# hannes-holey/GaPFlow

Measured on AMD Instinct MI355X. Metric: Mcell-updates/s (fp64), 4096^2 grid, higher is better.
Workload: dtype f64; 1 GPU; 2D journal bearing 4096x4096, fixed DH EOS, all-periodic, adaptive CFL 0.5 (BASELINE.json configs[2]); slabs=1

## Files before the change

gapflow_amd/csrc/api.hip:

```cpp
#include <hip/hip_runtime.h>
#include <algorithm>
#include <cmath>
#include <cstdio>
#include <cstdlib>
#include <cstring>
#include <map>
#include <mutex>
#include <string>
#include <tuple>
#include <vector>

#include "../../include/gapflow_hip.h"
#include "phys_setup.hpp"
#include "step_kernel.hip"
#include "aux_kernels.hip"
#include "step2_kernel.hip"
#include "gp_kernels.hip"
#include "elastic_kernels.hip"
#include "probe_kernels.hip"
#include "small_kernel.hip"
#include "profile_kernels.hip"
#include "checkpoint_kernels.hip"

using namespace gpf;
// ... 90 lines not shown
             double2* greens = nullptr; double2* spec = nullptr; double* dense = nullptr;
             double* u_prev = nullptr; double* h0 = nullptr; double* deformation = nullptr; } el;
    struct { bool on = false; int px = 0, py = 0, nky = 0, nranks = 1, relative = 0;
             int row0 = 0, nrows = 0, k0 = 0, nk = 0, nret = 0, nrows_all = 0, nmain = 0, main_g0 = 0, seam_side = -1, seam_g0 = 0, ref_row = -1;
             double alpha = 1.0, scale = 1.0;
             void* plan_y = nullptr; void* plan_x = nullptr; void* plan_yb = nullptr; int nxg = 0, g_lo = 0;
             double* dense = nullptr; double2* spec = nullptr; double2* send1 = nullptr; double2* recv1 = nullptr; double2* xspec = nullptr;
             double2* greens = nullptr; double2* send2 = nullptr; double2* recv2 = nullptr; double2* line = nullptr; double* ureal = nullptr;
             double* u_prev = nullptr; double* h0 = nullptr; double* deformation = nullptr; double* ref = nullptr; int* rows_all = nullptr; } els;
    double* gptile = nullptr;
    size_t gptile_doubles = 0;
    void* blas = nullptr;
    bool step_open = false;
    int open_parity = 0;
    bool has_q = false, has_topo = false, pre_run_done = false;
    bool prev_state_valid = false;
    long long fields_step = -1;
    bool fields_restored = false;
    long long host_step = 0;
    long long next_step = 0;
    Strip2Geom geom2[2];
    int nchunks2 = 0, nblocks2 = 0, npartials2_cap = 0, nblock_partials_cap = 0;
    bool plan2_valid = false;
    int nt_policy2 = 0;
    int keep_rows2 = 0;
    StepState* st_trial = nullptr;
    double* plan_master = nullptr;
    char plan2_note[400] = "";
};

static int enter(gpf_handle* h, bool reads_only) {
    HIP_TRY(hipSetDevice(h->cfg.device));
    if (!reads_only) { h->gp_state_mean_valid = false; h->fields_restored = false; }
    return GPF_OK;
}

static void make_phys(const gpf_config& c, Phys& P) {
    setup_phys(P, c.U, c.V, c.eta, c.zeta, c.dx, c.dy, c.eos, c.eos_par, c.piezo, c.piezo_par, c.thinning, c.thinning_par);
}

static int blocks_for(long long n, int bs = 256, int cap = 4096) {
    long long b = (n + bs - 1) / bs;
    return (int)std::max<long long>(1, std::min<long long>(b, cap));
}

#ifdef GPF_ONLY_EOS_DH
#define EOS_DISPATCH(eos, ...)                                                                          \
    do {                                                                                                \
        if ((eos) == GPF_EOS_DH) { constexpr int EOS_ = EOS_DH; __VA_ARGS__; }       \
    } while (0)
#else
// ... 62 lines not shown
    if (cfg->eos != GPF_EOS_DH) return fail(GPF_ERR_INVALID, "gpf_create: this build (-DGPF_ONLY_EOS_DH) holds the Dowson-Higginson kernels only");
#endif
    int ndev = 0;
    if (hipGetDeviceCount(&ndev) != hipSuccess || ndev == 0)
        return fail(GPF_ERR_NO_DEVICE, "gpf_create: no HIP device visible (this library has no CPU path)");
    if (cfg->device < 0 || cfg->device >= ndev) return fail(GPF_ERR_INVALID, "gpf_create: device ordinal out of range");
    HIP_TRY(hipSetDevice(cfg->device));

    gpf_handle* h = new gpf_handle();
    h->cfg = *cfg;
    Layout& L = h->L;
    L.Nx = cfg->Nx; L.Ny = cfg->Ny; L.off = 15;
    L.pitch = ((cfg->Ny + 2 + L.off + 15) / 16) * 16;
    if (const char* s = std::getenv("GPF_PITCH_PAD")) L.pitch += (std::atoi(s) / 16) * 16;
    L.plane = (long long)(cfg->Nx + 2) * L.pitch;
    if (const char* s = std::getenv("GPF_PLANE_PAD")) L.plane += (std::atoll(s) & ~1ll);
    for (int e = 0; e < 4; ++e) {
        for (int c = 0; c < 3; ++c) h->E.rule[e][c] = cfg->bc_rule[e][c];
        h->E.value[e] = cfg->bc_value[e];
    }
    h->E.halo[0] = cfg->halo_lo; h->E.halo[1] = cfg->halo_hi;
    h->split_edges = std::getenv("GPF_STEP_UNFUSED_EDGES") != nullptr;
    if (const char* s = std::getenv("GPF_ROWCOEF_TABLE")) h->rowcoef_table = std::atoi(s) != 0;
    h->gp_reuse_state_mean = std::getenv("GPF_GP_NO_STATE_MEAN") == nullptr;
    make_phys(*cfg, h->P);

    const size_t plane_b = (size_t)L.plane * sizeof(double);
    auto cleanup = [&](int code) { gpf_destroy(h); return code; };
#define HIP_TRY_C(expr)                                                                                 \
    do {                                                                                                \
        hipError_t e_ = (expr);                                                                         \
        if (e_ != hipSuccess)                                                                           \
            return cleanup(fail(GPF_ERR_HIP, std::string(#expr) + ": " + hipGetErrorString(e_)));      \
    } while (0)
    h->field_bytes = (3 * plane_b + PLANE_PAD_BYTES + 255) & ~(size_t)255;
    for (int b = 0; b < 2; ++b) {
        HIP_TRY_C(field_malloc((void**)&h->q[b], h->field_bytes));
        if (field_zero(0, h->q[b], h->field_bytes) != GPF_OK) { gpf_destroy(h); return GPF_ERR_HIP; }
    }
    HIP_TRY_C(field_malloc((void**)&h->topo, h->field_bytes));
    if (field_zero(0, h->topo, h->field_bytes) != GPF_OK) { gpf_destroy(h); return GPF_ERR_HIP; }
    HIP_TRY_C(hipDeviceSynchronize());
    const size_t g1n = (size_t)3 * L.pitch + (size_t)3 * (L.Nx + 2);
    HIP_TRY_C(hipMalloc(&h->g1, g1n * sizeof(double)));
    HIP_TRY_C(hipMemset(h->g1, 0, g1n * sizeof(double)));
    HIP_TRY_C(hipMalloc(&h->st, sizeof(StepState)));
// ... 413 lines not shown
    RowCoef* fresh = nullptr;
    if (source == 1) {
        HIP_TRY(hipMalloc(&fresh, (size_t)(n + 4) * sizeof(RowCoef)));
        HIP_TRY(hipMemsetAsync(fresh, 0, (size_t)(n + 4) * sizeof(RowCoef), h->stream));
        const double* col = h->topo + L.off + 1;
        hipLaunchKernelGGL(k_row_coef_table, dim3((n + 255) / 256), dim3(256), 0, h->stream, col, col + L.plane, (long long)L.pitch, n, h->P, fresh);
        for (int e = 0; e < 2; ++e) {
            if (!h->has_seam[e]) continue;
            const double* t = h->seam + (size_t)e * 8 * L.pitch + L.off + 1;
            hipLaunchKernelGGL(k_row_coef_table, dim3(1), dim3(64), 0, h->stream, t, t + L.pitch, 4ll * L.pitch, 2, h->P, fresh + n + 2 * e);
        }
        src = fresh;
    }
    hipError_t e = hipGetLastError();
    if (e == hipSuccess) e = hipMemcpyAsync(host, src, count * sizeof(double), hipMemcpyDeviceToHost, h->stream);
    if (e == hipSuccess) e = hipStreamSynchronize(h->stream);
    if (fresh) hipFree(fresh);
    if (e != hipSuccess) return fail(GPF_ERR_HIP, std::string("gpf_row_coefficients: ") + hipGetErrorString(e));
    return GPF_OK;
}

typedef void (*step2_kernel_t)(const Step2Args, const Phys);

static step2_kernel_t step2_kernel(int eos, bool has_ls, bool piezo, int D, int topo_mode) {
    step2_kernel_t k = nullptr;
    EOS_DISPATCH(eos, {
        if (piezo) {
            if (has_ls) k = D > 0 ? k_step2<EOS_, true, true, 1, 0> : k_step2<EOS_, true, true, -1, 0>;
            else k = D > 0 ? k_step2<EOS_, false, true, 1, 0> : k_step2<EOS_, false, true, -1, 0>;
        } else if (has_ls) {
            k = D > 0 ? k_step2<EOS_, true, false, 1, 0> : k_step2<EOS_, true, false, -1, 0>;
        } else if (topo_mode == 1) {
            k = D > 0 ? k_step2<EOS_, false, false, 1, 1> : k_step2<EOS_, false, false, -1, 1>;
        } else if (topo_mode == 2) {
            k = D > 0 ? k_step2<EOS_, false, false, 1, 2> : k_step2<EOS_, false, false, -1, 2>;
        } else if (topo_mode == 3) {
            k = D > 0 ? k_step2<EOS_, false, false, 1, 3> : k_step2<EOS_, false, false, -1, 3>;
        } else if (topo_mode == 4) {
            k = D > 0 ? k_step2<EOS_, false, false, 1, 4> : k_step2<EOS_, false, false, -1, 4>;
        } else {
            k = D > 0 ? k_step2<EOS_, false, false, 1, 0> : k_step2<EOS_, false, false, -1, 0>;
        }
    });
    return k;
}

static Strip2Geom strip2_geom(const Layout& L, int D) {
    Strip2Geom G;
// ... 77 lines not shown
    Step2Args a2;
    fill_step2_args(h, a2, D, honor_stop, log_base, slab_out, p2p);
    const bool slab = slab_out != nullptr;
    FinishArgs f;
    f.partials = h->partials; f.st = h->st;
    f.log = h->log; f.log_base = log_base; f.log_cap = h->log_cap; f.out = slab_out; f.honor_stop = honor_stop;
    f.L = L; f.E = h->E;
    f.p2p = p2p_args(h, p2p);
    f.arrive = h->arrive; f.msg = slab ? h->halo : nullptr;
    f.nstep_partials = np_step; f.block_partials = h->block_partials;
    GhostFillArgs gf;
    gf.qa = h->q[0]; gf.qb = h->q[1]; gf.st = h->st;
    gf.L = L; gf.E = h->E; gf.honor_stop = honor_stop;

    const int ntiles = (L.Nx + L.Ny + 63) / 64;
    const dim3 ggrid(std::min(ntiles, 512));
    const int nsend = slab ? std::min((6 * L.pitch + 1023) / 1024, 256) : 0;
    WaitArgs w;
    w.qa = h->q[0]; w.qb = h->q[1]; w.st = h->st; w.log = h->log; w.log_base = log_base; w.log_cap = h->log_cap;
    w.L = L; w.E = h->E; w.honor_stop = honor_stop; w.arrive = h->arrive + 1; w.timeout_ticks = h->p2p_timeout_ticks; w.p2p = f.p2p;
    w.gathered = nullptr; w.msg_len = 0; w.nranks = 0; w.rank_lo = w.rank_hi = -1; w.stage1 = fused ? 0 : 1;
    const bool has_ls = h->Ls != nullptr;
    if (fused) {
        const step2_kernel_t k2 = step2_kernel(h->cfg.eos, h->Ls != nullptr, h->cfg.piezo != 0, D, topo_mode_of(h));
        if (ev0) hipEventRecord(ev0, h->stream);
        hipLaunchKernelGGL(k2, dim3(h->nblocks2), dim3(256), 0, h->stream, a2, h->P);
        if (ev1) hipEventRecord(ev1, h->stream);
        if (p2p) {
            const dim3 cgrid(SLAB_COMMIT_BLOCKS);
            EOS_DISPATCH(h->cfg.eos, {
                hipLaunchKernelGGL((k_begin_slab<EOS_, false, false, false, true>), cgrid, dim3(256), 0, h->stream, g, w, h->P);
            });
        }
        h->g1_ready = false;
        HIP_TRY(hipGetLastError());
        return GPF_OK;
    }
    EOS_DISPATCH(h->cfg.eos, {
        if (!h->g1_ready) {
            if (topo_xonly(h)) hipLaunchKernelGGL((k_ghost_stage1<EOS_, false, false, true>), ggrid, dim3(256), 0, h->stream, g, h->P);
            else LS_PIEZO_DISPATCH(has_ls, h->cfg.piezo != 0, hipLaunchKernelGGL((k_ghost_stage1<EOS_, LS_, PZ_, false>), ggrid, dim3(256), 0, h->stream, g, h->P));
        }
        if (ev0) hipEventRecord(ev0, h->stream);
        hipLaunchKernelGGL(step2_kernel(h->cfg.eos, h->Ls != nullptr, h->cfg.piezo != 0, D, topo_mode_of(h)), dim3(h->nblocks2), dim3(256), 0, h->stream, a2, h->P);
        if (ev1) hipEventRecord(ev1, h->stream);
        hipLaunchKernelGGL((k_ghost_fill<EOS_>), dim3(h->nghost_blocks + nsend), dim3(256), 0, h->stream, gf, f, h->nghost_blocks, h->P);
        if (p2p) {
            if (topo_xonly(h)) hipLaunchKernelGGL((k_begin_slab<EOS_, false, false, true, true>), ggrid, dim3(256), 0, h->stream, g, w, h->P);
            else LS_PIEZO_DISPATCH(has_ls, h->cfg.piezo != 0, hipLaunchKernelGGL((k_begin_slab<EOS_, LS_, PZ_, false, true>), ggrid, dim3(256), 0, h->stream, g, w, h->P));
        }
    });
    h->g1_ready = p2p;
    HIP_TRY(hipGetLastError());
    return GPF_OK;
}

#include "api_probes.inc"

static bool small_grid_eligible(gpf_handle* h) {
    static const bool off = getenv("GPF_SMALL_GRID") && atoi(getenv("GPF_SMALL_GRID")) == 0;
    const long long nc = (long long)(h->L.Nx + 2) * (h->L.Ny + 2);
    return !off && nc * SMALL_DOUBLES_PER_CELL * 8 <= 150 * 1024 && h->cfg.thinning == GPF_THINNING_NONE && !h->E.halo[0] && !h->E.halo[1] &&
           !h->gp[0].set && !h->gp[1].set && !h->gp[2].set && !h->el.on;
}

static int enqueue_small_steps(gpf_handle* h, int nsteps, int honor_stop, long long log_base) {
    const Layout& L = h->L;
// ... 101 lines not shown
```

gapflow_amd/csrc/api_plan.inc:

```

constexpr int K2_LONG_MARCH_ROWS = 100;

static int plan_apply(gpf_handle* h, int nchunks, int nt, int keep = 0) {
    const Layout& L = h->L;
    const int nstrips = std::max(h->geom2[0].nstrips, h->geom2[1].nstrips);
    nchunks = std::max(1, std::min(nchunks, std::max(1, L.Nx / 4)));
    h->nchunks2 = nchunks;
    h->nt_policy2 = nt;
    h->keep_rows2 = nt >= 1 ? std::max(0, std::min(7, keep)) : 0;
    const int nwaves = nstrips * nchunks;
    h->nblocks2 = (((nwaves + 3) / 4) + 7) / 8 * 8;
    if (nwaves > h->npartials2_cap) {
        if (h->partials) HIP_TRY(hipFree(h->partials));
        h->partials = nullptr;
        HIP_TRY(hipMalloc(&h->partials, (size_t)nwaves * sizeof(Partial)));
        HIP_TRY(hipMemset(h->partials, 0, (size_t)nwaves * sizeof(Partial)));
        h->npartials2_cap = nwaves;
    }
    if (h->nblocks2 > h->nblock_partials_cap) {
        const int cap = std::max(1024, h->nblocks2);
        if (h->block_partials) HIP_TRY(hipFree(h->block_partials));
        h->block_partials = nullptr;
        HIP_TRY(hipMalloc(&h->block_partials, (size_t)cap * sizeof(Partial)));
        h->nblock_partials_cap = cap;
    }
    return GPF_OK;
}

static void fill_step2_args(gpf_handle* h, Step2Args& a2, int D, int honor_stop, long long log_base, double* slab_out, bool p2p);

static int plan_trial(gpf_handle* h, int D, float* us, int reps = 6, bool both = false) {
    static const int parity_value[2] = {0, 1};
    if (!h->st_trial) HIP_TRY(hipMalloc(&h->st_trial, sizeof(StepState)));
    h->prev_state_valid = false;
    both = both && h->plan_master != nullptr;
    int par = 0;
    if (both) GPF_TRY(current_parity(h, &par));
    Step2Args a2;
    fill_step2_args(h, a2, D, 0, 0, nullptr, false);
    a2.st = h->st_trial; a2.log = nullptr;
    const step2_kernel_t k2 = step2_kernel(h->cfg.eos, h->Ls != nullptr, h->cfg.piezo != 0, D, topo_mode_of(h));
    hipEvent_t e0, e1;
    HIP_TRY(hipEventCreate(&e0)); HIP_TRY(hipEventCreate(&e1));
    float total = 0.f;
    for (int r = -1; r < reps; ++r) {
        HIP_TRY(hipMemcpyAsync(h->st_trial, h->st, sizeof(StepState), hipMemcpyDeviceToDevice, h->stream));
        if (both && ((r + 1) & 1))
            HIP_TRY(hipMemcpyAsync(&h->st_trial->parity, &parity_value[par ^ 1], sizeof(int), hipMemcpyHostToDevice, h->stream));
        HIP_TRY(hipEventRecord(e0, h->stream));
        hipLaunchKernelGGL(k2, dim3(h->nblocks2), dim3(256), 0, h->stream, a2, h->P);
        HIP_TRY(hipEventRecord(e1, h->stream));
        HIP_TRY(hipEventSynchronize(e1));
        float ms = 0.f;
        HIP_TRY(hipEventElapsedTime(&ms, e0, e1));
        if (r >= 0) total += ms;
    }
    hipEventDestroy(e0); hipEventDestroy(e1);
    if (both) GPF_TRY(field_copy(h->stream, h->q[par], h->plan_master, h->field_bytes));
    HIP_TRY(hipGetLastError());
    *us = total / reps * 1e3f;
    return GPF_OK;
}

static float placement_best_seen(const gpf_handle* h, int D, float mine) {
// ... 109 lines not shown
        }
        h->topo = best_home;
    }
    GPF_TRY(trial(bi, bj, &us, true));
    HIP_TRY(hipStreamSynchronize(h->stream));
    for (double* b : rest) field_free(b);
    h->q[par] = pool[bi]; h->q[par ^ 1] = pool[bj];
    return GPF_OK;
}

static const char* const NT_NAME[3] = {"plain loads and stores", "non-temporal stores", "non-temporal loads and stores"};
constexpr int K2_KEEP_ROWS_DEFAULT = 4;
static const int K2_KEEP_CANDIDATES[2] = {3, 4};
static std::string keep_note(const gpf_handle* h) {
    if (h->nt_policy2 < 1) return "";
    char buf[64];
    std::snprintf(buf, sizeof buf, ", keep %d/8 rows on-die", h->keep_rows2);
    return buf;
}
static const char* coef_note(const gpf_handle* h) {
    const int topo = topo_mode_of(h);
    return topo == 4 ? ", row coefficients from the table" : topo == 3 ? ", row coefficients evaluated in the kernel" : "";
}
static int plan_step2(gpf_handle* h, int D) {
    if (h->plan2_valid) return GPF_OK;
    const Layout& L = h->L;
    h->geom2[0] = strip2_geom(L, 1);
    h->geom2[1] = strip2_geom(L, -1);
    const int nstrips = std::max(h->geom2[0].nstrips, h->geom2[1].nstrips);
    int per_cu = 0, ncu = 0;
    HIP_TRY(hipOccupancyMaxActiveBlocksPerMultiprocessor(&per_cu, (const void*)step2_kernel(h->cfg.eos, h->Ls != nullptr, h->cfg.piezo != 0, 1, topo_mode_of(h)), 256, 0));
    HIP_TRY(hipDeviceGetAttribute(&ncu, hipDeviceAttributeMultiprocessorCount, h->cfg.device));
    const int all_resident = std::max(1, std::max(1, per_cu * ncu) * 4 / nstrips);
    const int one_per_simd = (ncu * 4) / nstrips;
    const double streamed = (double)L.plane * 8.0 * (6 + (topo_mode_of(h) == 0 ? 3 : 0) + (h->Ls ? 1 : 0));
    const bool nt_possible = streamed > 192.0 * 1024 * 1024;
    const char* env_chunks = std::getenv("GPF_CHUNKS");
    const char* env_nt = std::getenv("GPF_NT") ? std::getenv("GPF_NT") : std::getenv("GPF_NT_STORES");
    const char* env_tune = std::getenv("GPF_PLAN_TUNE");
    int nchunks = all_resident;
    if (one_per_simd >= 1 && L.Nx / one_per_simd >= K2_LONG_MARCH_ROWS) nchunks = one_per_simd;
    int nt = nt_possible ? 2 : 0;
    if (env_chunks && std::atoi(env_chunks) > 0) nchunks = std::atoi(env_chunks);
    if (env_nt) nt = std::max(0, std::min(2, std::atoi(env_nt)));
    const char* env_keep = std::getenv("GPF_KEEP_ROWS");
    int keep = nt_possible ? K2_KEEP_ROWS_DEFAULT : 0;
    if (env_keep) keep = std::max(0, std::min(7, std::atoi(env_keep)));
    const bool tune = !(env_tune && std::atoi(env_tune) == 0) && !h->split_edges && h->pre_run_done && (long long)L.Nx * L.Ny >= (1ll << 20) &&
                      one_per_simd >= 1 && L.Nx / one_per_simd >= 16 && !(env_chunks && env_nt);
    if (!tune) {
        GPF_TRY(plan_apply(h, nchunks, nt, keep));
        std::snprintf(h->plan2_note, sizeof h->plan2_note, "%d chunks per strip, %s%s%s (rule of thumb%s)", h->nchunks2,
                      NT_NAME[h->nt_policy2], coef_note(h), keep_note(h).c_str(), (env_chunks || env_nt || env_keep) ? ", pinned by the environment" : "");
        h->plan2_valid = true;
        return GPF_OK;
    }
    std::string placement_note;
    GPF_TRY(plan_apply(h, nchunks, nt));
    {
        int par = 0;
        GPF_TRY(current_parity(h, &par));
        if (field_malloc((void**)&h->plan_master, h->field_bytes) == hipSuccess)
            GPF_TRY(field_copy(h->stream, h->plan_master, h->q[par], h->field_bytes));
        else { (void)hipGetLastError(); h->plan_master = nullptr; }
    }
    {
        float unused = 0.f;
        const double step_s = 1.1e-11 * (double)L.Nx * L.Ny + 1e-5;
        GPF_TRY(plan_trial(h, D, &unused, (int)std::min(200.0, std::max(8.0, 0.012 / step_s))));
    }
    float best = 0.f;
    int best_chunks = nchunks;
    int best_nt = nt;
    int best_keep = 0;
    std::string seen, keep_seen;
    auto pick_plan = [&]() -> int {
        best = 0.f;
        seen.clear();
        for (int c : {one_per_simd, all_resident}) {
            if (env_chunks && std::atoi(env_chunks) > 0) c = std::atoi(env_chunks);
            for (int pol = 0; pol < (nt_possible && !env_nt ? 3 : 1); ++pol) {
                const int cand_nt = env_nt ? nt : pol;
                GPF_TRY(plan_apply(h, c, cand_nt));
                float us = 0.f;
                GPF_TRY(plan_trial(h, D, &us, 6, true));
                char buf[48];
                std::snprintf(buf, sizeof buf, " %d/%s %.0f", h->nchunks2, cand_nt == 2 ? "nt" : cand_nt == 1 ? "nts" : "plain", us);
                seen += buf;
                if (best == 0.f || us < best) { best = us; best_chunks = c; best_nt = cand_nt; }
            }
            if ((env_chunks && std::atoi(env_chunks) > 0) || one_per_simd == all_resident) break;
        }
        best_keep = 0;
        keep_seen.clear();
        if (best_nt >= 1) {
            if (env_keep) best_keep = keep;
            else if (nt_possible) {
                char buf[48];
                std::snprintf(buf, sizeof buf, " 0 %.0f", best);
                keep_seen = buf;
                float best_k = best;
                for (int k : K2_KEEP_CANDIDATES) {
                    GPF_TRY(plan_apply(h, best_chunks, best_nt, k));
                    float us = 0.f;
                    GPF_TRY(plan_trial(h, D, &us, 6, true));
                    std::snprintf(buf, sizeof buf, ", %d %.0f", k, us);
                    keep_seen += buf;
                    if (us < best_k) { best_k = us; best_keep = k; }
                }
            }
        }
        return plan_apply(h, best_chunks, best_nt, best_keep);
    };
    const bool verify = std::getenv("GPF_PLACEMENT_PRINT") && std::atoi(std::getenv("GPF_PLACEMENT_PRINT")) >= 2;
    auto stamp = [&](const char* when) {
        if (!verify) return;
        int par = 0;
        if (current_parity(h, &par) != GPF_OK) return;
        std::fprintf(stderr, "[gpf] %-28s q[par] %p %016llx   master %p %016llx\n", when, (void*)h->q[par], field_checksum(h->stream, h->q[par], h->field_bytes),
                     (void*)h->plan_master, h->plan_master ? field_checksum(h->stream, h->plan_master, h->field_bytes) : 0ull);
    };
    stamp("before the first plan");
    GPF_TRY(pick_plan());
    stamp("after the first plan");
    const std::string first_seen = seen;
    GPF_TRY(plan_placement(h, D, placement_note));
    stamp("after the placement");
    if (!placement_note.empty()) GPF_TRY(pick_plan());
    stamp("after the second plan");
    HIP_TRY(hipStreamSynchronize(h->stream));
    field_free(h->plan_master);
    h->plan_master = nullptr;
    GPF_TRY(plan_apply(h, best_chunks, best_nt, best_keep));
    const std::string kept = keep_note(h) + (keep_seen.empty() ? (env_keep && h->nt_policy2 >= 1 ? " (pinned by the environment)" : "")
                                                               : " (timed, us: k" + keep_seen + ")");
    std::snprintf(h->plan2_note, sizeof h->plan2_note, "%d chunks per strip, %s%s%s (timed, us:%s;%s%s%s)", h->nchunks2,
                  NT_NAME[h->nt_policy2], coef_note(h), kept.c_str(), seen.c_str(), placement_note.c_str(),
                  placement_note.empty() ? "" : "; before the placement:", placement_note.empty() ? "" : first_seen.c_str());
    DBG("plan_step2: %s", h->plan2_note);
    h->plan2_valid = true;
    return GPF_OK;
}

extern "C" const char* gpf_plan_note(gpf_handle* h) { return h ? h->plan2_note : ""; }
```

gapflow_amd/csrc/step2_kernel.hip:

```cpp
#include <hip/hip_runtime.h>
#include "device_types.hpp"

namespace gpf {

constexpr int STRIP2 = 126;
#ifndef GPF_K2_AHEAD
#define GPF_K2_AHEAD 2
#endif
#ifndef GPF_K2_AHEAD_LINE
#define GPF_K2_AHEAD_LINE 4
#endif
#ifndef GPF_K2_MINWAVES
#define GPF_K2_MINWAVES 2
#endif
#ifndef GPF_K2_MINWAVES_LINE
#define GPF_K2_MINWAVES_LINE GPF_K2_MINWAVES
#endif
template <int EOS, bool HAS_LS, bool PIEZO>
struct Step2Weight {
    static constexpr bool heavy = EOS == EOS_PL || EOS == EOS_MT || EOS == EOS_BWR || EOS == EOS_BAYADA || (HAS_LS && PIEZO);
};

struct Strip2Geom {
    int w0;
// ... 61 lines not shown
template <int N>
__device__ __forceinline__ void asm_wait3(dpair& a, dpair& b, dpair& c) {
    asm volatile("s_waitcnt vmcnt(%3)" : "+v"(a), "+v"(b), "+v"(c) : "n"(N) : "memory");
}
template <int N>
__device__ __forceinline__ void asm_wait1(dpair& a) {
    asm volatile("s_waitcnt vmcnt(%1)" : "+v"(a) : "n"(N) : "memory");
}

__device__ __forceinline__ double uniform_load(const double* p) {
    typedef const __attribute__((address_space(4))) double* cptr;
    return *(cptr)(unsigned long long)p;
}

__device__ __forceinline__ RowCoef uniform_load_coef(const RowCoef* p) {
    typedef double d8 __attribute__((ext_vector_type(8)));
    typedef const __attribute__((address_space(4))) d8* cptr;
    const d8 v = *(cptr)(unsigned long long)p;
    RowCoef r;
    r.A = v[0]; r.B = v[1]; r.C = v[2]; r.S0 = v[3]; r.S1a = v[4]; r.S1b = v[5]; r.S2a = v[6]; r.S2b = v[7];
    return r;
}

template <int TOPO, bool HAS_LS>
struct RawRow {
    dpair q[3];
    dpair t[TOPO == 0 ? 3 : 1];
    dpair ls[HAS_LS ? 1 : 1];
    double th, thx, thy;
};

struct Row2 { double rho[2], jx[2], jy[2], h[2], hx[2], hy[2], Ls[2]; };

template <int EOS>
struct Red {
    double ekin, v2, c2;
    int flags;
    __device__ __forceinline__ void init() { ekin = 0.0; v2 = 0.0; c2 = (EOS == EOS_DH) ? __builtin_inf() : 0.0; flags = 0; }
    __device__ __forceinline__ void cell(double r, double jx, double jy, double w, const Phys& P) {
        const double v = (jx * jx + jy * jy) * rcp(r);
        ekin += w * (v * 0.5);
        v2 = fmax(v2, v);
        if (v != v) flags |= 1;
        if (r < 0.0) flags |= 2;
        if (EOS == EOS_DH) {
            c2 = fmin(c2, fabs(P.e[7] - r));
        } else {
            const double c = eos_c2<EOS>(r, P);
            if (!(c >= 0.0)) flags |= 4;
            c2 = fmax(c2, c);
        }
    }
};

template <int EOS, bool HAS_LS, bool PIEZO, int D, int TOPO>
__device__ __forceinline__ void step_strip2(const Step2Args& a, const Phys& P, const double* __restrict__ qin,
                                            double* __restrict__ qout, int strip, int chunk, int lane,
                                            double (*stash)[128], Acc& result) {
    const Layout L = a.L;
    const Strip2Geom G = a.G;
    const bool fused = (a.fused & 1) != 0;
    const int policy = __builtin_amdgcn_readfirstlane(a.fused);

    const bool y_periodic = a.E.rule[2][0] == BC_P;
    const bool ghost_strip = strip == G.s_ghost;
    const bool wrap_strip = fused && y_periodic && ghost_strip;
    const bool wrap_lane = wrap_strip && (lane == G.lane_wrap || lane == G.lane_wrap + 1);
    const int ma = wrap_lane ? G.wrap_ma + 2 * (lane - G.lane_wrap) : G.w0 + strip * STRIP2 + 2 * lane;
    const int iy_lo_raw = D > 0 ? ma : L.Ny - ma;
    const bool lane_ok = iy_lo_raw >= -1 && iy_lo_raw <= L.Ny + 1;
    const int iy_lo = lane_ok ? iy_lo_raw : -1;
    const int iy0 = D > 0 ? iy_lo : iy_lo + 1, iy1 = D > 0 ? iy_lo + 1 : iy_lo;
    const bool out0 = lane_ok && !wrap_lane && lane >= 1 && ma >= 1 && ma <= L.Ny;
    const bool out1 = lane_ok && !wrap_lane && lane <= 62 && ma + 1 >= 1 && ma + 1 <= L.Ny;
    const bool is_ghost_lane = ghost_strip && lane == G.lane_ghost;
    const int gsrc_lane = y_periodic ? G.wrap_src_lane : (G.slot_ghost ? G.lane_ghost : G.lane_ghost - 1);
    const int gsrc_slot = y_periodic ? G.wrap_src_slot : (G.slot_ghost ? 0 : 1);

// ... 78 lines not shown
                         : "v"(a0), "v"(a1), "v"(a2), "v"(a3), "v"(a4), "v"(a5), [nt] "s"(policy & 4) : "memory", "scc");
        } else if constexpr (HAS_LS) {
            const double* const a3 = (dummy ? lane_q : lane_ls) + rb;
            asm volatile(GPF_ROW_HEAD GPF_LD(0, 4) GPF_LD(1, 5) GPF_LD(2, 6) GPF_LD(3, 7) GPF_ROW_MID
                         GPF_LDNT(0, 4) GPF_LDNT(1, 5) GPF_LDNT(2, 6) GPF_LDNT(3, 7) GPF_ROW_TAIL
                         : "=&v"(r.q[0]), "=&v"(r.q[1]), "=&v"(r.q[2]), "=&v"(r.ls[0])
                         : "v"(a0), "v"(a1), "v"(a2), "v"(a3), [nt] "s"(policy & 4) : "memory", "scc");
        } else {
            asm volatile(GPF_ROW_HEAD GPF_LD(0, 3) GPF_LD(1, 4) GPF_LD(2, 5) GPF_ROW_MID GPF_LDNT(0, 3) GPF_LDNT(1, 4) GPF_LDNT(2, 5) GPF_ROW_TAIL
                         : "=&v"(r.q[0]), "=&v"(r.q[1]), "=&v"(r.q[2])
                         : "v"(a0), "v"(a1), "v"(a2), [nt] "s"(policy & 4) : "memory", "scc");
        }
#undef GPF_LD
#undef GPF_LDNT
#undef GPF_ROW_HEAD
#undef GPF_ROW_MID
#undef GPF_ROW_TAIL
        if (TOPO == 1 || TOPO == 3) {
            r.th = uniform_load(a.topo_line + ix); r.thx = uniform_load(a.topo_line + (L.Nx + 2) + ix);
            r.thy = TOPO == 1 ? uniform_load(a.topo_line + 2 * (L.Nx + 2) + ix) : 0.0;
        }
    };
    constexpr bool HEAVY = Step2Weight<EOS, HAS_LS, PIEZO>::heavy;
    constexpr int AHEAD_ROWS = PIEZO ? 1 : ((TOPO == 3 || TABLE) ? (HEAVY ? 2 : GPF_K2_AHEAD_LINE) : GPF_K2_AHEAD);
#ifndef GPF_K2_COUNT_STORES
#define GPF_K2_COUNT_STORES 1
#endif
    const bool stores_every_row = GPF_K2_COUNT_STORES && __builtin_amdgcn_ballot_w64(out0 || out1) != 0ull;
    auto arrive = [&](Raw& r, const int n) {
        constexpr int LOOSE = AHEAD_ROWS * NL, EXACT = AHEAD_ROWS * (NL + 3);
        static_assert(EXACT <= 63, "vmcnt is a 6-bit counter");
        const int exact = __builtin_amdgcn_readfirstlane((stores_every_row && n > n_first + AHEAD_ROWS) ? 1 : 0);
#define GPF_WAIT_ROW "s_cmp_lg_u32 %[ex], 0\n\ts_cbranch_scc1 .Lgpf_exact_%=\n\ts_waitcnt vmcnt(%[loose])\n.Lgpf_exact_%=:\n\ts_waitcnt vmcnt(%[exact])"
        if constexpr (TOPO == 0 && HAS_LS)
            asm volatile(GPF_WAIT_ROW : "+v"(r.q[0]), "+v"(r.q[1]), "+v"(r.q[2]), "+v"(r.t[0]), "+v"(r.t[1]), "+v"(r.t[2]), "+v"(r.ls[0])
                         : [ex] "s"(exact), [loose] "n"(LOOSE), [exact] "n"(EXACT) : "memory", "scc");
        else if constexpr (TOPO == 0)
            asm volatile(GPF_WAIT_ROW : "+v"(r.q[0]), "+v"(r.q[1]), "+v"(r.q[2]), "+v"(r.t[0]), "+v"(r.t[1]), "+v"(r.t[2])
                         : [ex] "s"(exact), [loose] "n"(LOOSE), [exact] "n"(EXACT) : "memory", "scc");
        else if constexpr (HAS_LS)
            asm volatile(GPF_WAIT_ROW : "+v"(r.q[0]), "+v"(r.q[1]), "+v"(r.q[2]), "+v"(r.ls[0])
                         : [ex] "s"(exact), [loose] "n"(LOOSE), [exact] "n"(EXACT) : "memory", "scc");
        else
            asm volatile(GPF_WAIT_ROW : "+v"(r.q[0]), "+v"(r.q[1]), "+v"(r.q[2])
                         : [ex] "s"(exact), [loose] "n"(LOOSE), [exact] "n"(EXACT) : "memory", "scc");
#undef GPF_WAIT_ROW
    };
// ... 200 lines not shown
                }
                const int ixo = D > 0 ? n - 1 : L.Nx + 2 - n;
                const long long rbo = (long long)ixo * L.pitch;
#if GPF_K2_NT & 2
                const bool store_nt = (policy & 2) && (ixo & 7) >= ((policy >> 3) & 7);
#endif
                auto st16 = [&](double* __restrict__ rowp, double va, double vb) {
                    dpair v;
                    v.x = D > 0 ? va : vb; v.y = D > 0 ? vb : va;
                    dpair* p = reinterpret_cast<dpair*>(reinterpret_cast<char*>(rowp) + lane_bytes);
#if GPF_K2_NT & 2
                    asm volatile("s_cmp_lg_u32 %[nt], 0\n\ts_cbranch_scc1 .Lgpf_stnt_%=\n\t"
                                 "global_store_dwordx4 %0, %1, off\n\ts_branch .Lgpf_stdone_%=\n"
                                 ".Lgpf_stnt_%=:\n\tglobal_store_dwordx4 %0, %1, off nt\n"
                                 ".Lgpf_stdone_%=:\n\ts_nop 0"
                                 :: "v"(p), "v"(v), [nt] "s"(__builtin_amdgcn_readfirstlane(store_nt ? 1 : 0)) : "memory", "scc");
#else
                    *p = v;
#endif
                };
                auto st8 = [&](double* __restrict__ rowp, unsigned int bytes, double v) {
                    *reinterpret_cast<double*>(reinterpret_cast<char*>(rowp) + bytes) = v;
                };
                if (out0 && out1) {
                    st16(qo0 + rbo, o[0][0], o[1][0]); st16(qo1 + rbo, o[0][1], o[1][1]); st16(qo2 + rbo, o[0][2], o[1][2]);
                } else if (out0) {
                    const unsigned int b = (unsigned int)(L.off + iy0) * 8u;
                    st8(qo0 + rbo, b, o[0][0]); st8(qo1 + rbo, b, o[0][1]); st8(qo2 + rbo, b, o[0][2]);
                } else if (out1) {
                    const unsigned int b = (unsigned int)(L.off + iy1) * 8u;
                    st8(qo0 + rbo, b, o[1][0]); st8(qo1 + rbo, b, o[1][1]); st8(qo2 + rbo, b, o[1][2]);
                }
                const double w = 1.0 + (ixo == seam_row_lo ? 1.0 : 0.0) + (ixo == seam_row_hi ? 1.0 : 0.0);
                if (out0) red.cell(o[0][0], o[0][1], o[0][2], w, P);
                if (out1) red.cell(o[1][0], o[1][1], o[1][2], w, P);
            }
            for (int k = 0; k < 2; ++k) {
                part[k][0] = (cur.rho[k] + q1[k][0]) - dt * (-cx * q1[k][1] + cy * (dn[k][0] - gy[k][0]) - g[k].s0);
                part[k][1] = (cur.jx[k] + q1[k][1]) - dt * (-cx * g[k].fx1 + cy * (dn[k][1] - gy[k][1]) - g[k].s1);
                part[k][2] = (cur.jy[k] + q1[k][2]) - dt * (-cx * g[k].fx2 + cy * (dn[k][2] - gy[k][2]) - g[k].s2);
            }
        }
        if (TABLE) rc_row = coef_of(n + 1);
    };
    for (int n = n_first - 1;;) {
        march(n, rowbuf[0], rowbuf[AHEAD]); if (++n > n_last + 1) break;
        march(n, rowbuf[1], rowbuf[0]); if (++n > n_last + 1) break;
// ... 84 lines not shown
            }
        }
        if (a.p2p.on) asm volatile("s_waitcnt vmcnt(0)" ::: "memory");
    }
#endif

    for (int s = 32; s >= 1; s >>= 1) {
        red.ekin += __shfl_down(red.ekin, s);
        red.v2 = fmax(red.v2, __shfl_down(red.v2, s));
        const double oc = __shfl_down(red.c2, s);
        red.c2 = (EOS == EOS_DH) ? fmin(red.c2, oc) : fmax(red.c2, oc);
        red.flags |= __shfl_down(red.flags, s);
    }
    if (EOS == EOS_DH) {
        const double it = rcp(red.c2);
        red.c2 = (red.c2 == __builtin_inf()) ? 0.0 : P.e[6] * (it * it);
    }
#ifdef GPF_K2_NO_POSTPASS
    red.flags = 0;
#endif
    result.ekin = red.ekin; result.v2 = red.v2; result.c2 = red.c2; result.mass = 0.0; result.flags = red.flags;
}

template <int EOS, bool HAS_LS, bool PIEZO, int D, int TOPO>
__global__ __launch_bounds__(256, (Step2Weight<EOS, HAS_LS, PIEZO>::heavy ? 1 : ((TOPO == 1 || TOPO == 3 || TOPO == 4) ? GPF_K2_MINWAVES_LINE : GPF_K2_MINWAVES)))
void k_step2(const Step2Args a, const Phys P) {
    __shared__ double stash[4][3][128];
    __shared__ Acc red_sm[4];
    __shared__ int s_last;
    if (halted(a.st, a.honor_stop)) return;
    if (predictor_direction(a.st) != D) __builtin_trap();
    const int par = a.st->parity;
    const double* qin = par ? a.qb : a.qa;
    double* qout = const_cast<double*>(par ? a.qa : a.qb);

    const int nb = gridDim.x;
    const int lb = (int)(blockIdx.x & 7) * (nb >> 3) + (int)(blockIdx.x >> 3);
    const int wv = __builtin_amdgcn_readfirstlane(threadIdx.x >> 6), lane = threadIdx.x & 63;
    const int w = lb * 4 + wv;
    const int strip = w % a.G.nstrips, chunk = w / a.G.nstrips;
    const bool active = chunk < a.nchunks;

    Acc own;
    own.zero();
    if (active) step_strip2<EOS, HAS_LS, PIEZO, D, TOPO>(a, P, qin, qout, strip, chunk, lane, stash[wv], own);

    if (!(a.fused & 1)) {
        if (active && lane == 0) {
            Partial p;
            p.ekin = own.ekin; p.vmax2 = own.v2; p.c2max = own.c2; p.flags = (double)own.flags;
            a.partials[w] = p;
        }
        return;
    }
#ifdef GPF_K2_NO_FINISH
    if (blockIdx.x == 0 && threadIdx.x == 0) commit_step(a.st, own.ekin + 1.0, own.v2, own.c2, own.flags, a.log, a.log_base, a.log_cap);
    return;
#endif
    if (lane == 0) red_sm[wv] = own;
    __syncthreads();
    if (threadIdx.x == 0) {
        Acc tot = red_sm[0];
        for (int i = 1; i < 4; ++i) { tot.ekin += red_sm[i].ekin; tot.v2 = fmax(tot.v2, red_sm[i].v2); tot.c2 = fmax(tot.c2, red_sm[i].c2); tot.flags |= red_sm[i].flags; }
        publish_partial(a.block_partials + blockIdx.x, tot);
        const unsigned int t = __hip_atomic_fetch_add(a.arrive, 1u, GPF_ORDER_ARRIVE, __HIP_MEMORY_SCOPE_AGENT);
        s_last = (t == (unsigned int)nb - 1) ? 1 : 0;
        if (s_last) __hip_atomic_store(a.arrive, 0u, __ATOMIC_RELAXED, __HIP_MEMORY_SCOPE_AGENT);
    }
// ... 7 lines not shown
```

Measured before the change: 122,800 Mcell-updates/s.

## Add three-waves-per-SIMD step2 kernel variant and include it in autotuning

Adds a variant of the step2 kernel with a launch-bounds minimum of three waves per SIMD, for the light x-only-gap topology modes. It shortens the row lookahead and rebuilds the output pointers from one wave-uniform base to save registers. The planner adds this form to the timed candidates, with a chunk count chosen to avoid power-of-two aliasing. It also loosens the tuning threshold. Higher occupancy is meant to hide memory latency better, at the risk of register spills or less lookahead.

```diff
diff --git a/gapflow_amd/csrc/api.hip b/gapflow_amd/csrc/api.hip
--- a/gapflow_amd/csrc/api.hip
+++ b/gapflow_amd/csrc/api.hip
@@ -136,11 +136,13 @@
     Strip2Geom geom2[2];
     int nchunks2 = 0, nblocks2 = 0, npartials2_cap = 0, nblock_partials_cap = 0;
     bool plan2_valid = false;
+    int waves2 = 0;
+    int waves_pin = 0;
     int nt_policy2 = 0;
     int keep_rows2 = 0;
     StepState* st_trial = nullptr;
     double* plan_master = nullptr;
-    char plan2_note[400] = "";
+    char plan2_note[640] = "";
 };
 
 static int enter(gpf_handle* h, bool reads_only) {
@@ -249,6 +251,7 @@
     h->E.halo[0] = cfg->halo_lo; h->E.halo[1] = cfg->halo_hi;
     h->split_edges = std::getenv("GPF_STEP_UNFUSED_EDGES") != nullptr;
     if (const char* s = std::getenv("GPF_ROWCOEF_TABLE")) h->rowcoef_table = std::atoi(s) != 0;
+    if (const char* s = std::getenv("GPF_K2_WAVES")) h->waves_pin = std::max(0, std::min(3, std::atoi(s)));
     h->gp_reuse_state_mean = std::getenv("GPF_GP_NO_STATE_MEAN") == nullptr;
     make_phys(*cfg, h->P);
 
@@ -708,8 +711,21 @@
 
 typedef void (*step2_kernel_t)(const Step2Args, const Phys);
 
-static step2_kernel_t step2_kernel(int eos, bool has_ls, bool piezo, int D, int topo_mode) {
+template <int EOS, int D, int TOPO>
+static step2_kernel_t step2_kernel_three_waves() {
+    if constexpr (Step2Weight<EOS, false, false>::heavy) return nullptr;
+    else return k_step2<EOS, false, false, D, TOPO, 3>;
+}
+
+static step2_kernel_t step2_kernel(int eos, bool has_ls, bool piezo, int D, int topo_mode, int waves = 0) {
     step2_kernel_t k = nullptr;
+    if (waves == 3 && !has_ls && !piezo && (topo_mode == 3 || topo_mode == 4)) {
+        EOS_DISPATCH(eos, {
+            if (topo_mode == 3) k = D > 0 ? step2_kernel_three_waves<EOS_, 1, 3>() : step2_kernel_three_waves<EOS_, -1, 3>();
+            else k = D > 0 ? step2_kernel_three_waves<EOS_, 1, 4>() : step2_kernel_three_waves<EOS_, -1, 4>();
+        });
+        if (k) return k;
+    }
     EOS_DISPATCH(eos, {
         if (piezo) {
             if (has_ls) k = D > 0 ? k_step2<EOS_, true, true, 1, 0> : k_step2<EOS_, true, true, -1, 0>;
@@ -833,7 +849,7 @@
     w.gathered = nullptr; w.msg_len = 0; w.nranks = 0; w.rank_lo = w.rank_hi = -1; w.stage1 = fused ? 0 : 1;
     const bool has_ls = h->Ls != nullptr;
     if (fused) {
-        const step2_kernel_t k2 = step2_kernel(h->cfg.eos, h->Ls != nullptr, h->cfg.piezo != 0, D, topo_mode_of(h));
+        const step2_kernel_t k2 = step2_kernel(h->cfg.eos, h->Ls != nullptr, h->cfg.piezo != 0, D, topo_mode_of(h), h->waves2);
         if (ev0) hipEventRecord(ev0, h->stream);
         hipLaunchKernelGGL(k2, dim3(h->nblocks2), dim3(256), 0, h->stream, a2, h->P);
         if (ev1) hipEventRecord(ev1, h->stream);
@@ -853,7 +869,7 @@
             else LS_PIEZO_DISPATCH(has_ls, h->cfg.piezo != 0, hipLaunchKernelGGL((k_ghost_stage1<EOS_, LS_, PZ_, false>), ggrid, dim3(256), 0, h->stream, g, h->P));
         }
         if (ev0) hipEventRecord(ev0, h->stream);
-        hipLaunchKernelGGL(step2_kernel(h->cfg.eos, h->Ls != nullptr, h->cfg.piezo != 0, D, topo_mode_of(h)), dim3(h->nblocks2), dim3(256), 0, h->stream, a2, h->P);
+        hipLaunchKernelGGL(step2_kernel(h->cfg.eos, h->Ls != nullptr, h->cfg.piezo != 0, D, topo_mode_of(h), h->waves2), dim3(h->nblocks2), dim3(256), 0, h->stream, a2, h->P);
         if (ev1) hipEventRecord(ev1, h->stream);
         hipLaunchKernelGGL((k_ghost_fill<EOS_>), dim3(h->nghost_blocks + nsend), dim3(256), 0, h->stream, gf, f, h->nghost_blocks, h->P);
         if (p2p) {
diff --git a/gapflow_amd/csrc/api_plan.inc b/gapflow_amd/csrc/api_plan.inc
--- a/gapflow_amd/csrc/api_plan.inc
+++ b/gapflow_amd/csrc/api_plan.inc
@@ -4,7 +4,9 @@
 static int plan_apply(gpf_handle* h, int nchunks, int nt, int keep = 0) {
     const Layout& L = h->L;
     const int nstrips = std::max(h->geom2[0].nstrips, h->geom2[1].nstrips);
-    nchunks = std::max(1, std::min(nchunks, std::max(1, L.Nx / 4)));
+    const char* const env_pinned = std::getenv("GPF_CHUNKS");
+    const int min_rows = (env_pinned && std::atoi(env_pinned) > 0) ? 3 : 4;
+    nchunks = std::max(1, std::min(nchunks, std::max(1, L.Nx / min_rows)));
     h->nchunks2 = nchunks;
     h->nt_policy2 = nt;
     h->keep_rows2 = nt >= 1 ? std::max(0, std::min(7, keep)) : 0;
@@ -39,7 +41,7 @@
     Step2Args a2;
     fill_step2_args(h, a2, D, 0, 0, nullptr, false);
     a2.st = h->st_trial; a2.log = nullptr;
-    const step2_kernel_t k2 = step2_kernel(h->cfg.eos, h->Ls != nullptr, h->cfg.piezo != 0, D, topo_mode_of(h));
+    const step2_kernel_t k2 = step2_kernel(h->cfg.eos, h->Ls != nullptr, h->cfg.piezo != 0, D, topo_mode_of(h), h->waves2);
     hipEvent_t e0, e1;
     HIP_TRY(hipEventCreate(&e0)); HIP_TRY(hipEventCreate(&e1));
     float total = 0.f;
@@ -195,6 +197,15 @@
     const int topo = topo_mode_of(h);
     return topo == 4 ? ", row coefficients from the table" : topo == 3 ? ", row coefficients evaluated in the kernel" : "";
 }
+static bool chunks_alias(const Layout& L, int nchunks) {
+    if (nchunks < 2 || L.Nx % nchunks != 0) return false;
+    const double mib = (double)(L.Nx / nchunks) * L.pitch * 8.0 / (1024.0 * 1024.0);
+    if (mib < 0.98) return false;
+    const double p2 = std::exp2(std::round(std::log2(mib)));
+    return std::fabs(mib - p2) <= 0.02 * p2;
+}
+static const char* form_note(const gpf_handle* h) { return h->waves2 == 3 ? ", three-wave form" : ", one- / two-wave form"; }
+
 static int plan_step2(gpf_handle* h, int D) {
     if (h->plan2_valid) return GPF_OK;
     const Layout& L = h->L;
@@ -206,6 +217,18 @@
     HIP_TRY(hipDeviceGetAttribute(&ncu, hipDeviceAttributeMultiprocessorCount, h->cfg.device));
     const int all_resident = std::max(1, std::max(1, per_cu * ncu) * 4 / nstrips);
     const int one_per_simd = (ncu * 4) / nstrips;
+    const int topo = topo_mode_of(h);
+    const step2_kernel_t k3 = step2_kernel(h->cfg.eos, h->Ls != nullptr, h->cfg.piezo != 0, 1, topo, 3);
+    const bool has_three = k3 != step2_kernel(h->cfg.eos, h->Ls != nullptr, h->cfg.piezo != 0, 1, topo);
+    int three_resident = 0;
+    if (has_three) {
+        int per_cu3 = 0;
+        HIP_TRY(hipOccupancyMaxActiveBlocksPerMultiprocessor(&per_cu3, (const void*)k3, 256, 0));
+        three_resident = std::max(1, std::max(1, per_cu3 * ncu) * 4 / nstrips);
+        while (three_resident > 1 && chunks_alias(L, three_resident)) --three_resident;
+    }
+    const int pin = (h->waves_pin == 3 && !has_three) ? 0 : h->waves_pin;
+    const char* const pin_ignored = (h->waves_pin == 3 && !has_three) ? ", GPF_K2_WAVES=3 ignored: this kernel has no three-wave form" : "";
     const double streamed = (double)L.plane * 8.0 * (6 + (topo_mode_of(h) == 0 ? 3 : 0) + (h->Ls ? 1 : 0));
     const bool nt_possible = streamed > 192.0 * 1024 * 1024;
     const char* env_chunks = std::getenv("GPF_CHUNKS");
@@ -214,17 +237,22 @@
     int nchunks = all_resident;
     if (one_per_simd >= 1 && L.Nx / one_per_simd >= K2_LONG_MARCH_ROWS) nchunks = one_per_simd;
     int nt = nt_possible ? 2 : 0;
+    h->waves2 = pin == 3 ? 3 : 0;
+    if (pin == 1 && one_per_simd >= 1) nchunks = one_per_simd;
+    else if (pin == 2) nchunks = all_resident;
+    else if (pin == 3) nchunks = three_resident;
     if (env_chunks && std::atoi(env_chunks) > 0) nchunks = std::atoi(env_chunks);
     if (env_nt) nt = std::max(0, std::min(2, std::atoi(env_nt)));
     const char* env_keep = std::getenv("GPF_KEEP_ROWS");
     int keep = nt_possible ? K2_KEEP_ROWS_DEFAULT : 0;
     if (env_keep) keep = std::max(0, std::min(7, std::atoi(env_keep)));
     const bool tune = !(env_tune && std::atoi(env_tune) == 0) && !h->split_edges && h->pre_run_done && (long long)L.Nx * L.Ny >= (1ll << 20) &&
-                      one_per_simd >= 1 && L.Nx / one_per_simd >= 16 && !(env_chunks && env_nt);
+                      one_per_simd >= 1 && L.Nx / one_per_simd >= 8 && !(env_chunks && env_nt);
     if (!tune) {
         GPF_TRY(plan_apply(h, nchunks, nt, keep));
-        std::snprintf(h->plan2_note, sizeof h->plan2_note, "%d chunks per strip, %s%s%s (rule of thumb%s)", h->nchunks2,
-                      NT_NAME[h->nt_policy2], coef_note(h), keep_note(h).c_str(), (env_chunks || env_nt || env_keep) ? ", pinned by the environment" : "");
+        std::snprintf(h->plan2_note, sizeof h->plan2_note, "%d chunks per strip%s, %s%s%s (rule of thumb%s%s)", h->nchunks2, form_note(h),
+                      NT_NAME[h->nt_policy2], coef_note(h), keep_note(h).c_str(), (env_chunks || env_nt || env_keep || pin) ? ", pinned by the environment" : "",
+                      pin_ignored);
         h->plan2_valid = true;
         return GPF_OK;
     }
@@ -246,24 +274,37 @@
     int best_chunks = nchunks;
     int best_nt = nt;
     int best_keep = 0;
+    int best_waves = h->waves2;
     std::string seen, keep_seen;
+    std::vector<std::pair<int, int>> forms;
+    {
+        const int fixed = env_chunks ? std::atoi(env_chunks) : 0;
+        auto add = [&](int c, int waves) {
+            const std::pair<int, int> f(fixed > 0 ? fixed : c, waves);
+            if (std::find(forms.begin(), forms.end(), f) == forms.end()) forms.push_back(f);
+        };
+        if (pin == 0 || pin == 1) add(one_per_simd, 0);
+        if (pin == 0 || pin == 2) add(all_resident, 0);
+        if (has_three && (pin == 0 || pin == 3)) add(three_resident, 3);
+    }
     auto pick_plan = [&]() -> int {
         best = 0.f;
         seen.clear();
-        for (int c : {one_per_simd, all_resident}) {
-            if (env_chunks && std::atoi(env_chunks) > 0) c = std::atoi(env_chunks);
+        for (const std::pair<int, int>& form : forms) {
+            const int c = form.first;
+            h->waves2 = form.second;
             for (int pol = 0; pol < (nt_possible && !env_nt ? 3 : 1); ++pol) {
                 const int cand_nt = env_nt ? nt : pol;
                 GPF_TRY(plan_apply(h, c, cand_nt));
                 float us = 0.f;
                 GPF_TRY(plan_trial(h, D, &us, 6, true));
                 char buf[48];
-                std::snprintf(buf, sizeof buf, " %d/%s %.0f", h->nchunks2, cand_nt == 2 ? "nt" : cand_nt == 1 ? "nts" : "plain", us);
+                std::snprintf(buf, sizeof buf, " %d%s/%s %.0f", h->nchunks2, form.second == 3 ? "w3" : "", cand_nt == 2 ? "nt" : cand_nt == 1 ? "nts" : "plain", us);
                 seen += buf;
-                if (best == 0.f || us < best) { best = us; best_chunks = c; best_nt = cand_nt; }
+                if (best == 0.f || us < best) { best = us; best_chunks = c; best_nt = cand_nt; best_waves = form.second; }
             }
-            if ((env_chunks && std::atoi(env_chunks) > 0) || one_per_simd == all_resident) break;
-        }
+        }
+        h->waves2 = best_waves;
         best_keep = 0;
         keep_seen.clear();
         if (best_nt >= 1) {
@@ -304,12 +345,14 @@
     HIP_TRY(hipStreamSynchronize(h->stream));
     field_free(h->plan_master);
     h->plan_master = nullptr;
+    h->waves2 = best_waves;
     GPF_TRY(plan_apply(h, best_chunks, best_nt, best_keep));
     const std::string kept = keep_note(h) + (keep_seen.empty() ? (env_keep && h->nt_policy2 >= 1 ? " (pinned by the environment)" : "")
                                                                : " (timed, us: k" + keep_seen + ")");
-    std::snprintf(h->plan2_note, sizeof h->plan2_note, "%d chunks per strip, %s%s%s (timed, us:%s;%s%s%s)", h->nchunks2,
+    std::snprintf(h->plan2_note, sizeof h->plan2_note, "%d chunks per strip%s, %s%s%s (timed, us:%s;%s%s%s)%s%s", h->nchunks2, form_note(h),
                   NT_NAME[h->nt_policy2], coef_note(h), kept.c_str(), seen.c_str(), placement_note.c_str(),
-                  placement_note.empty() ? "" : "; before the placement:", placement_note.empty() ? "" : first_seen.c_str());
+                  placement_note.empty() ? "" : "; before the placement:", placement_note.empty() ? "" : first_seen.c_str(),
+                  pin ? " (waves per SIMD pinned by the environment)" : "", pin_ignored);
     DBG("plan_step2: %s", h->plan2_note);
     h->plan2_valid = true;
     return GPF_OK;
diff --git a/gapflow_amd/csrc/step2_kernel.hip b/gapflow_amd/csrc/step2_kernel.hip
--- a/gapflow_amd/csrc/step2_kernel.hip
+++ b/gapflow_amd/csrc/step2_kernel.hip
@@ -107,6 +107,13 @@
     return r;
 }
 
+template <typename T>
+__device__ __forceinline__ T* uniform_ptr(T* p) {
+    const unsigned long long b = (unsigned long long)p;
+    const unsigned int lo = __builtin_amdgcn_readfirstlane((unsigned int)b), hi = __builtin_amdgcn_readfirstlane((unsigned int)(b >> 32));
+    return (T*)(((unsigned long long)hi << 32) | lo);
+}
+
 template <int TOPO, bool HAS_LS>
 struct RawRow {
     dpair q[3];
@@ -138,7 +145,7 @@
     }
 };
 
-template <int EOS, bool HAS_LS, bool PIEZO, int D, int TOPO>
+template <int EOS, bool HAS_LS, bool PIEZO, int D, int TOPO, int WAVES = 0>
 __device__ __forceinline__ void step_strip2(const Step2Args& a, const Phys& P, const double* __restrict__ qin,
                                             double* __restrict__ qout, int strip, int chunk, int lane,
                                             double (*stash)[128], Acc& result) {
@@ -263,7 +270,7 @@
         }
     };
     constexpr bool HEAVY = Step2Weight<EOS, HAS_LS, PIEZO>::heavy;
-    constexpr int AHEAD_ROWS = PIEZO ? 1 : ((TOPO == 3 || TABLE) ? (HEAVY ? 2 : GPF_K2_AHEAD_LINE) : GPF_K2_AHEAD);
+    constexpr int AHEAD_ROWS = PIEZO ? 1 : ((TOPO == 3 || TABLE) ? (HEAVY ? 2 : (WAVES == 3 ? 2 : GPF_K2_AHEAD_LINE)) : GPF_K2_AHEAD);
 #ifndef GPF_K2_COUNT_STORES
 #define GPF_K2_COUNT_STORES 1
 #endif
@@ -510,7 +517,20 @@
                 auto st8 = [&](double* __restrict__ rowp, unsigned int bytes, double v) {
                     *reinterpret_cast<double*>(reinterpret_cast<char*>(rowp) + bytes) = v;
                 };
-                if (out0 && out1) {
+                if constexpr (WAVES == 3) {
+                    double* const ob0 = uniform_ptr(qo0 + rbo);
+                    double* const ob1 = ob0 + L.plane;
+                    double* const ob2 = ob0 + 2 * L.plane;
+                    if (out0 && out1) {
+                        st16(ob0, o[0][0], o[1][0]); st16(ob1, o[0][1], o[1][1]); st16(ob2, o[0][2], o[1][2]);
+                    } else if (out0) {
+                        const unsigned int b = (unsigned int)(L.off + iy0) * 8u;
+                        st8(ob0, b, o[0][0]); st8(ob1, b, o[0][1]); st8(ob2, b, o[0][2]);
+                    } else if (out1) {
+                        const unsigned int b = (unsigned int)(L.off + iy1) * 8u;
+                        st8(ob0, b, o[1][0]); st8(ob1, b, o[1][1]); st8(ob2, b, o[1][2]);
+                    }
+                } else if (out0 && out1) {
                     st16(qo0 + rbo, o[0][0], o[1][0]); st16(qo1 + rbo, o[0][1], o[1][1]); st16(qo2 + rbo, o[0][2], o[1][2]);
                 } else if (out0) {
                     const unsigned int b = (unsigned int)(L.off + iy0) * 8u;
@@ -641,9 +661,11 @@
     result.ekin = red.ekin; result.v2 = red.v2; result.c2 = red.c2; result.mass = 0.0; result.flags = red.flags;
 }
 
-template <int EOS, bool HAS_LS, bool PIEZO, int D, int TOPO>
-__global__ __launch_bounds__(256, (Step2Weight<EOS, HAS_LS, PIEZO>::heavy ? 1 : ((TOPO == 1 || TOPO == 3 || TOPO == 4) ? GPF_K2_MINWAVES_LINE : GPF_K2_MINWAVES)))
+template <int EOS, bool HAS_LS, bool PIEZO, int D, int TOPO, int WAVES = 0>
+__global__ __launch_bounds__(256, (WAVES > 0 ? WAVES : (Step2Weight<EOS, HAS_LS, PIEZO>::heavy ? 1 : ((TOPO == 1 || TOPO == 3 || TOPO == 4) ? GPF_K2_MINWAVES_LINE : GPF_K2_MINWAVES))))
 void k_step2(const Step2Args a, const Phys P) {
+    static_assert(WAVES == 0 || (WAVES == 3 && (TOPO == 3 || TOPO == 4) && !HAS_LS && !PIEZO && !Step2Weight<EOS, HAS_LS, PIEZO>::heavy),
+                  "three waves per SIMD: the light x-only-gap kernels only");
     __shared__ double stash[4][3][128];
     __shared__ Acc red_sm[4];
     __shared__ int s_last;
@@ -662,7 +684,7 @@
 
     Acc own;
     own.zero();
-    if (active) step_strip2<EOS, HAS_LS, PIEZO, D, TOPO>(a, P, qin, qout, strip, chunk, lane, stash[wv], own);
+    if (active) step_strip2<EOS, HAS_LS, PIEZO, D, TOPO, WAVES>(a, P, qin, qout, strip, chunk, lane, stash[wv], own);
 
     if (!(a.fused & 1)) {
         if (active && lane == 0) {
```

Measured after the change: 120,100 Mcell-updates/s. 0.978x the previous value.
